# pacellie/raytracer_challenge

Hardware: AMD Instinct MI355X
Metric: Mrays/s (unique rays: primary+shadow+reflection+refraction) at 1920x1080 depth-5 (higher is better)
Workload: dtype f64

## Files before the change

include/rtc.h:

```cpp
#ifndef RTC_H
#define RTC_H
#include <stddef.h>
#include <stdint.h>
#ifdef __cplusplus
extern "C" {
#endif

typedef struct rtc_scene rtc_scene;

enum {
  RTC_OK = 0,
  RTC_ERR_INVALID = 1,
  RTC_ERR_UNSUPPORTED = 2,
  RTC_ERR_DEVICE = 3,
  RTC_ERR_NAN = 4
};

enum { RTC_SPHERE = 0, RTC_PLANE = 1, RTC_CUBE = 2, RTC_CYLINDER = 3, RTC_CONE = 4, RTC_TRIANGLE = 5, RTC_SMOOTH_TRIANGLE = 6 };
enum { RTC_FLAG_CASTS_SHADOW = 1u, RTC_FLAG_CLOSED = 2u };

typedef struct rtc_prim {
  int32_t geometry;
  uint32_t flags;
  int32_t material;
// ... 305 lines not shown
                      uint32_t* order, uint32_t order_cap, uint64_t* keys, uint32_t keys_cap, int32_t* root, double* frame, int32_t* depth, int32_t* stack_need);
int rtc_bvh_collapse_raw(const void* nodes, uint32_t n_nodes, int32_t root, int32_t* depth, int32_t* stack_need);

int rtc_light_grid_build_raw(const int32_t* geometry, const double* limits, const double* transform_inv, const double* tris, uint32_t n_prims, const double* light, int32_t n,
                             int32_t max_list, int32_t tight, uint32_t* cells, uint32_t cells_cap, int32_t* items, uint32_t items_cap, uint32_t* n_items);

int rtc_scan_raw(rtc_scene* scene, uint64_t* values, uint64_t n, uint64_t* total);

enum { RTC_CULL_SLAB = 0, RTC_CULL_POINT = 1, RTC_CULL_GATE = 2, RTC_CULL_PLANE = 3, RTC_CULL_BEHIND = 4 };
int rtc_cull_probe_raw(rtc_scene* scene, int32_t kind, const double* records, uint64_t n, uint8_t* answers);

uint32_t rtc_scene_wavefront_lds_bytes(const rtc_scene*);

int rtc_scene_wavefront_ts_grid(const rtc_scene*, int32_t sync, uint32_t* grid, uint32_t* n_cu, uint32_t* spare_cus, uint32_t* live);

enum { RTC_TRACE_DEFAULT = 0, RTC_TRACE_COUNT = 1, RTC_TRACE_LEAN = 2, RTC_TRACE_3WAVE = 3 };
enum { RTC_WF_TS_MEM = 0, RTC_WF_TS_MEM_COUNT = 1, RTC_WF_TS_LDS = 2, RTC_WF_TS_LDS_COUNT = 3 };
enum { RTC_SHADE_COUNT = 0, RTC_SHADE_COUNT_UV = 1, RTC_SHADE_UV = 2, RTC_SHADE_PIPE_LV0 = 3, RTC_SHADE_PIPE = 4, RTC_SHADE_PAT = 5 };
typedef struct rtc_kernel_info {
  int32_t variant;
  int32_t n_kops;
  int32_t n_kplanes;
  int32_t n_kaux;
  int32_t has_recs;
  int32_t all_plain;
  int32_t no_glass_mirror;
  int32_t big_scene;
  uint32_t lds_bytes;
  int32_t trace_build;
  int32_t wf_ts_build;
// ... 14 lines not shown
```

raytracer_challenge_amd/csrc/device_scene.h:

```cpp
#pragma once
#include <stddef.h>
#include <stdint.h>

enum { OP_PRIM = 0, OP_GROUP = 1, OP_MESH = 2, OP_BVH = 3, OP_QUIRK = 4, OP_QGRID = 5, OP_CSG = 6, OP_CSG_END = 7 };

struct DOp {
  int32_t op, a, b, c;
  int32_t g;
  int32_t pad[3];
};

#define RTC_KOPS 12
#define RTC_KPLANES 6
struct DPlaneK {
  double row[4];
  int32_t prim;
  int32_t gcond;
  int32_t pad[2];
  double n[3];
};

struct DBvhNode {
  float lo0[3], hi0[3];
  float lo1[3], hi1[3];
// ... 216 lines not shown
  unsigned long long bx, by, bz;
  __builtin_memcpy(&bx, &x, 8); __builtin_memcpy(&by, &y, 8); __builtin_memcpy(&bz, &z, 8);
  return rtc_splitmix64(rtc_splitmix64(rtc_splitmix64(rtc_splitmix64((unsigned long long)(uint32_t)light) ^ bx) ^ by) ^ bz);
}
static inline RTC_HD double rtc_area_jitter(unsigned long long h, unsigned j) {
  return (double)(rtc_splitmix64(h ^ (unsigned long long)j) >> 11) * 0x1.0p-53;
}
#define RTC_ALIGHT 16
#define RTC_SLIGHT 22

#define RTC_WF_SHADE_COUNT 32
#define RTC_WF_OVERFLOW 63
#define RTC_WF_CHUNK_NEXT 64
#define RTC_WF_TOP_COUNT (64 + 32 * 8 * (RTC_MAX_FUEL + 2))
#define RTC_WF_SHADE_TOP_COUNT (RTC_WF_TOP_COUNT + 32)
#define RTC_WF_COUNTS (RTC_WF_TOP_COUNT + 64)
#ifndef RTC_WF_CHUNK
#define RTC_WF_CHUNK 64u
#endif
#define RTC_SR_PLAIN 0x40000000
#define RTC_WF_MISS (-2)
struct DWave {
  double* rq[2];
  double* h_t;
  int32_t* h_prim;
  double* h_n12;
  double* sr;
  int32_t* sr_mat;
  int32_t* sr_node;
  double* contrib;
  int32_t* child;
// ... 30 lines not shown
```

raytracer_challenge_amd/csrc/rtc_device.hpp:

```cpp
#pragma once

#include <hip/hip_runtime.h>
#include <stdint.h>

#include <algorithm>
#include <type_traits>

#include "background_point.h"
#include "device_scene.h"
#include "spot_factor.h"

#define EPS 0.00001
#ifndef RTC_BLOCK
#define RTC_BLOCK 64
#endif
#ifndef RTC_WAVES_PER_SIMD
#define RTC_WAVES_PER_SIMD 1
#endif
#ifdef RTC_TRAVERSE_NOINLINE
#define TRAVERSE_INLINE __noinline__
#else
#define TRAVERSE_INLINE __forceinline__
#endif
#ifndef RTC_LANE_ID
// ... 1872 lines not shown
constexpr RtcWfTsBuild rtc_pick_wf_ts_build(bool count, bool lds) { return lds ? (count ? RTC_TS_LDS_COUNT : RTC_TS_LDS) : (count ? RTC_TS_MEM_COUNT : RTC_TS_MEM); }
constexpr unsigned rtc_pick_wf_ts_lds_grid(int n_cu, int spare) {
  return (unsigned)(n_cu < 1 ? 1 : (spare <= 0 ? n_cu : (spare >= n_cu ? 1 : n_cu - spare)));
}
static_assert(rtc_pick_wf_ts_lds_grid(256, 0) == 256u && rtc_pick_wf_ts_lds_grid(256, 24) == 232u && rtc_pick_wf_ts_lds_grid(256, 255) == 1u, "n_cu - spare");
static_assert(rtc_pick_wf_ts_lds_grid(256, 256) == 1u && rtc_pick_wf_ts_lds_grid(256, 261) == 1u && rtc_pick_wf_ts_lds_grid(1, 1) == 1u, "spare >= n_cu: one block");
static_assert(rtc_pick_wf_ts_lds_grid(256, -8) == 256u && rtc_pick_wf_ts_lds_grid(0, 0) == 1u, "a negative spare: n_cu; never an empty grid");
constexpr int rtc_wf_spare_cus_default(int n_cu) { return n_cu < 8 ? 0 : 3 * (n_cu / 8); }
static_assert(rtc_wf_spare_cus_default(256) == 96 && rtc_wf_spare_cus_default(32) == 12 && rtc_wf_spare_cus_default(4) == 0, "3 / 8 of the CUs");
constexpr RtcWfShadeBuild rtc_pick_wf_shade_build(bool count, bool has_uv, bool all_plain, bool level0) {
  if (has_uv) return count ? RTC_SH_COUNT_UV : RTC_SH_UV;
  if (count) return RTC_SH_COUNT;
  if (all_plain) return level0 ? RTC_SH_PIPE_LV0 : RTC_SH_PIPE;
  return RTC_SH_PAT;
}
enum RtcWfShadeNpBuild { RTC_SH_NP = 0, RTC_SH_NP_COUNT = 1, RTC_SH_NP_UV = 2, RTC_SH_NP_COUNT_UV = 3 };
constexpr RtcWfShadeNpBuild rtc_pick_wf_shade_np_build(bool count, bool has_uv) {
  return has_uv ? (count ? RTC_SH_NP_COUNT_UV : RTC_SH_NP_UV) : (count ? RTC_SH_NP_COUNT : RTC_SH_NP);
}

enum RtcExt {
  RTC_EXT_NONE = 0,
  RTC_EXT_BG = 1,
  RTC_EXT_NP = 2,
  RTC_EXT_NP_BG = 3,
};
constexpr int RTC_N_EXT = 4;
constexpr bool rtc_ext_bg(int e) { return (e & RTC_EXT_BG) != 0; }
constexpr bool rtc_ext_np(int e) { return (e & RTC_EXT_NP) != 0; }
static inline RtcExt rtc_ext_of(const RtcSceneExt& X) { return (RtcExt)((X.bg ? RTC_EXT_BG : 0) | (X.bump ? RTC_EXT_NP : 0)); }
// ... 59 lines not shown
```

raytracer_challenge_amd/csrc/rtc_kernels.hip:

```cpp
#include <cstdio>
#include <cstdlib>
#include <utility>

#include "../../include/rtc.h"
#include "rtc_device.hpp"

#ifdef RTC_EMU
#include "rtc_feat.hip"
constexpr int RTC_VARIANTS_BUILT = 6;
#else
constexpr int RTC_VARIANTS_BUILT = RTC_N_VARIANTS;
#endif
template <int... V>
static const RtcVariantOps& rtc_ops(int v, std::integer_sequence<int, V...>) {
  static const RtcVariantOps ops[RTC_N_VARIANTS] = {rtc_variant_ops<V>()...};
  return ops[v];
}
static const RtcVariantOps& rtc_ops(int v) { return rtc_ops(v, std::make_integer_sequence<int, RTC_VARIANTS_BUILT>{}); }
static int rtc_variant(const DScene& S, bool wavefront) {
  return rtc_pick_variant(rtc_scene_feat(S), S.n_kops > 0, S.has_area != 0, S.has_uv != 0, S.has_spot != 0, wavefront);
}

#ifndef RTC_WF_SHADE_WAVES
#define RTC_WF_SHADE_WAVES 4
// ... 13 lines not shown
  const unsigned j = prim >= 0 ? wf_index(parts, W.cap, (unsigned)w) : (first < count ? wf_index(parts, W.cap, (unsigned)first) : 0u);
  WfShadeIn in = {prim, {0.0, 0.0, 0.0, 0.0, 0.0, 0.0}, 1.0, 0.0};
  if (!LV0) in.ray = wf_load_ray(W, level, j, in.weight);
  in.t = W.h_t[j];
  return in;
}
#ifndef RTC_EMU
__device__ __forceinline__ unsigned wf_row_scan16(unsigned v) {
  v += (unsigned)__builtin_amdgcn_update_dpp(0, (int)v, 0x111, 0xf, 0xf, true);
  v += (unsigned)__builtin_amdgcn_update_dpp(0, (int)v, 0x112, 0xf, 0xf, true);
  v += (unsigned)__builtin_amdgcn_update_dpp(0, (int)v, 0x114, 0xf, 0xf, true);
  v += (unsigned)__builtin_amdgcn_update_dpp(0, (int)v, 0x118, 0xf, 0xf, true);
  return v;
}
#endif
}
template <bool COUNT, bool PAT = true, bool UV = false, bool PIPE = false, bool LV0 = false, bool NP = false>
__global__ void __launch_bounds__(RTC_WF_SHADE_BLOCK, RTC_WF_SHADE_WAVES) wf_shade(std::conditional_t<NP, DSceneNp, DScene> S, DCamera cam, DPixelMap pm, DWave W, int level, unsigned n0, int fuel0, DStats* __restrict__ stats) {
  constexpr int end_of[5] = {0, 1, 2, 3, 3};
  constexpr int n_waves = RTC_WF_SHADE_BLOCK >= 64 ? RTC_WF_SHADE_BLOCK / 64 : 1;
  static_assert(n_waves <= 8, "wf_shade: eight counters per class");
  __shared__ unsigned s_cnt2[2][40];
  unsigned parity = 0;
  const WorkMap wm = make_workmap(pm, cam);
  const bool level0 = PIPE ? LV0 : level == 0;
  const WfParts parts = level0 ? WfParts{0u, n0} : wf_count(W, level, n0);
  const unsigned count = parts.top + parts.bottom;
  const size_t cap = W.cap;
  const double L = (double)S.n_lights;
  const int fuel = fuel0 - level;
  unsigned n_reflect = 0, n_refract = 0;
  int32_t* ch = W.child + (size_t)level * 2 * cap;
  double* nq = W.rq[(level + 1) & 1];
  const int lane = RTC_LANE_ID;
  const int wave = (int)(threadIdx.x / (RTC_WF_SHADE_BLOCK >= 64 ? 64 : 1));
  const unsigned long long step = (unsigned long long)gridDim.x * RTC_WF_SHADE_BLOCK;
  WfShadeIn nx = {-1, {0.0, 0.0, 0.0, 0.0, 0.0, 0.0}, 1.0, 0.0};
// ... 39 lines not shown
        if (S.pats[S.mat_pattern[P.mat]].tag != 1) {
          pattern_at<UV>(S, P, st, cr, cg, cbl);
          mat = P.mat;
        }
      }
    }
    const bool blend = hit && reflective > 0.0 && transparency > 0.0;
    double R = 0.0;
    if (blend) {
      R = blend_reflectance(st, n1, n2, fuel, cr, cg, cbl);
      if (R != R && mat < 0) mat = ~mat;
    }
    ChildRays spawn = {false, false, 0.0, 0.0, 0.0, 0.0, 0.0};
    if (hit && fuel > 0) spawn = child_rays(st, n1, n2, weight, L, reflective, transparency, blend, R);
    const unsigned long long lt = (1ull << lane) - 1ull;
    const bool on_plane = hit && geom == 1;
    const unsigned long long m_rec0 = __ballot(hit && on_plane ? 1 : 0), m_rec1 = __ballot(hit && !on_plane ? 1 : 0);
    const unsigned long long m_c0 = __ballot(spawn.refl && on_plane ? 1 : 0), m_c1 = __ballot(spawn.refl && !on_plane ? 1 : 0), m_c2 = __ballot(spawn.refr ? 1 : 0);
    unsigned* s_cnt = s_cnt2[parity];
    parity ^= 1u;
    if (lane == 0) {
      s_cnt[wave] = (unsigned)__popcll(m_rec0); s_cnt[8 + wave] = (unsigned)__popcll(m_rec1);
      s_cnt[16 + wave] = (unsigned)__popcll(m_c0); s_cnt[24 + wave] = (unsigned)__popcll(m_c1); s_cnt[32 + wave] = (unsigned)__popcll(m_c2);
    }
    if (PIPE) nx = wf_shade_prefetch<LV0>(W, parts, level, base + step + threadIdx.x, lane, count, nx_prim);
    __syncthreads();
#ifndef RTC_EMU
    if (PIPE && n_waves == 8 && wave == 0) {
      const unsigned c = lane < 40 ? s_cnt[lane] : 0u;
      const unsigned in_row = wf_row_scan16(c);
      const unsigned r0 = (unsigned)__builtin_amdgcn_readlane((int)in_row, 7), r01 = (unsigned)__builtin_amdgcn_readlane((int)in_row, 15);
      const unsigned k0 = (unsigned)__builtin_amdgcn_readlane((int)in_row, 23), k01 = (unsigned)__builtin_amdgcn_readlane((int)in_row, 31);
      const unsigned k2 = (unsigned)__builtin_amdgcn_readlane((int)in_row, 39);
      const unsigned t_rn = r0, t_rf = r01 - r0, t_cn = k0, t_cf = k01 - k0 + k2;
      const unsigned total = lane == 0 ? t_rn : lane == 1 ? t_rf : lane == 2 ? t_cn : t_cf;
      unsigned first = 0u;
      if (lane < 4 && total) {
        const int row = lane == 0 ? RTC_WF_SHADE_COUNT + level : lane == 1 ? RTC_WF_SHADE_TOP_COUNT + level : lane == 2 ? level + 1 : RTC_WF_TOP_COUNT + level + 1;
        const unsigned old = atomicAdd(&W.counts[row], total);
        const bool fits = (unsigned long long)old + total <= W.cap;
        if (!fits) { W.counts[RTC_WF_OVERFLOW] = 1u; stats->wf_overflow = 1ull; }
        first = (lane & 1) ? (fits ? W.cap - old - total : W.cap) : old;
      }
      const unsigned b_rn = (unsigned)__builtin_amdgcn_readlane((int)first, 0), b_rf = (unsigned)__builtin_amdgcn_readlane((int)first, 1);
      const unsigned b_cn = (unsigned)__builtin_amdgcn_readlane((int)first, 2), b_cf = (unsigned)__builtin_amdgcn_readlane((int)first, 3);
      if (lane < 40) {
        const unsigned ex = in_row - c;
        s_cnt[lane] = lane < 8 ? b_rn + ex : lane < 16 ? b_rf + ex - r0 : lane < 24 ? b_cn + ex : lane < 32 ? b_cf + ex - k0 : b_cf + k01 - k0 + ex;
      }
    }
    if (!PIPE || n_waves != 8)
#endif
    if (threadIdx.x == 0) {
      unsigned t[4] = {0u, 0u, 0u, 0u}, b[4];
      for (int k = 0; k < 5; k++)
        for (int w = 0; w < n_waves; w++) t[end_of[k]] += s_cnt[8 * k + w];
      const int row[4] = {RTC_WF_SHADE_COUNT + level, RTC_WF_SHADE_TOP_COUNT + level, level + 1, RTC_WF_TOP_COUNT + level + 1};
      for (int e = 0; e < 4; e++) {
        const unsigned old = t[e] ? atomicAdd(&W.counts[row[e]], t[e]) : 0u;
        const bool fits = (unsigned long long)old + t[e] <= W.cap;
        if (!fits) { W.counts[RTC_WF_OVERFLOW] = 1u; stats->wf_overflow = 1ull; }
        b[e] = (e & 1) ? (fits ? W.cap - old - t[e] : W.cap) : old;
      }
      for (int k = 0; k < 5; k++)
        for (int w = 0; w < n_waves; w++) { const unsigned r = s_cnt[8 * k + w]; s_cnt[8 * k + w] = b[end_of[k]]; b[end_of[k]] += r; }
    }
    __syncthreads();
    const unsigned s = on_plane ? s_cnt[wave] + (unsigned)__popcll(m_rec0 & lt) : s_cnt[8 + wave] + (unsigned)__popcll(m_rec1 & lt);
    const unsigned jr = on_plane ? s_cnt[16 + wave] + (unsigned)__popcll(m_c0 & lt) : s_cnt[24 + wave] + (unsigned)__popcll(m_c1 & lt);
    const unsigned jt = s_cnt[32 + wave] + (unsigned)__popcll(m_c2 & lt);
    if (hit && s < W.cap) {
      double* r = W.sr;
      r[s] = st.px; r[cap + s] = st.py; r[2 * cap + s] = st.pz;
      r[3 * cap + s] = st.nx; r[4 * cap + s] = st.ny; r[5 * cap + s] = st.nz;
      if (mat >= 0) {
        r[6 * cap + s] = cr; r[7 * cap + s] = cg; r[8 * cap + s] = cbl;
        W.sr_mat[s] = mat;
      } else {
        if (!PIPE) shading_row = (int)S.mat[8 * ~mat + 7];
        W.sr_mat[s] = RTC_SR_PLAIN | shading_row;
      }
      W.sr_node[s] = (int32_t)i;
    }
// ... 86 lines not shown
}
int rtc_ext_trace_build(const DScene& S, const RtcSceneExt& X) {
  return X.bump ? rtc_pick_np_build(S.has_area != 0, S.has_uv != 0, S.has_spot != 0, X.bg != nullptr) : rtc_pick_bg_build(S.has_area != 0, S.has_uv != 0, S.has_spot != 0);
}
bool rtc_scene_is_big(unsigned long long scene_bytes) { return rtc_big_scene(scene_bytes); }

#ifndef RTC_EMU

unsigned rtc_wavefront_grid(const DScene& S, int n_cu) {
  return (unsigned)std::max(1, n_cu * rtc_ops(rtc_variant(S, true)).wf_ts_blocks_per_cu(rtc_stack_bytes(S)));
}
unsigned rtc_wavefront_lds_grid(int n_cu, int spare) { return rtc_pick_wf_ts_lds_grid(n_cu, spare); }
int rtc_wavefront_spare_cus_default(int n_cu) { return rtc_wf_spare_cus_default(n_cu); }
#endif

uint64_t rtc_wavefront_work(const DCamera& cam, const DPixelMap& pm) {
  if (pm.mode == 2 && cam.hsize >= 8 && pm.n % cam.hsize == 0) return (uint64_t)((cam.hsize + 7) / 8) * ((pm.n / cam.hsize + 7) / 8) * 64;
  return pm.n;
}

#ifndef RTC_EMU
void rtc_launch_wf_background(const DScene& S, const DCamera& cam, const DPixelMap& pm, const DWave& W, int level, unsigned n0, const DBackground& bg, unsigned blocks,
                              hipStream_t stream);
#endif
void rtc_launch_wavefront(const DScene& S, const DCamera& cam, const DPixelMap& pm, int fuel, const DWave& W, double* rgb, double* hit_t, int* hit_prim, int* hit_k,
                          DStats* stats, bool count, hipStream_t stream, unsigned blocks, unsigned shade_blocks, unsigned lds, unsigned lds_blocks, const RtcSceneExt& X) {
  if (pm.n == 0) return;
  const RtcVariantOps& ops = rtc_ops(rtc_variant(S, true));
  const RtcFrame F = {S, cam, pm, hit_t, hit_prim, hit_k, stats, stream, count};
  const unsigned n0 = (unsigned)rtc_wavefront_work(cam, pm);
  const dim3 sgrid(std::max(1u, shade_blocks)), sblock(RTC_WF_SHADE_BLOCK);
  auto shade = [&](auto kernel, const auto& scene, int level) { hipLaunchKernelGGL(kernel, sgrid, sblock, 0, stream, scene, cam, pm, W, level, n0, fuel, stats); };
#ifndef RTC_EMU
  DSceneNp N;
  if (X.bump) N = rtc_widen_scene(S, X);
#endif
  for (int level = 0; level <= fuel + 1; level++) {
    const int tl = level <= fuel ? level : -1, sl = level - 1;
#ifndef RTC_EMU
    if (!lds || !ops.launch_wf_ts_lds(F, RtcLevel{W, tl, sl, n0, level, fuel - level, std::max(1u, lds_blocks), lds}))
#endif
    ops.launch_wf_ts(F, RtcLevel{W, tl, sl, n0, level, fuel - level, blocks, 0u});
    if (level > fuel) break;
#ifndef RTC_EMU
    if (X.bg) rtc_launch_wf_background(S, cam, pm, W, level, n0, *X.bg, 4u * std::max(1u, shade_blocks), stream);
    if (X.bump) {
      switch (rtc_pick_wf_shade_np_build(count, S.has_uv != 0)) {
        case RTC_SH_NP_COUNT_UV: shade(wf_shade<true, true, true, false, false, true>, N, level); break;
        case RTC_SH_NP_UV: shade(wf_shade<false, true, true, false, false, true>, N, level); break;
        case RTC_SH_NP_COUNT: shade(wf_shade<true, true, false, false, false, true>, N, level); break;
        case RTC_SH_NP: shade(wf_shade<false, true, false, false, false, true>, N, level); break;
      }
      continue;
    }
#endif
    switch (rtc_scene_shade_build(S, count, level == 0)) {
#ifndef RTC_EMU
      case RTC_SH_COUNT_UV: shade(wf_shade<true, true, true>, S, level); break;
      case RTC_SH_UV: shade(wf_shade<false, true, true>, S, level); break;
#else
      case RTC_SH_COUNT_UV: case RTC_SH_UV: break;
#endif
      case RTC_SH_COUNT: shade(wf_shade<true>, S, level); break;
      case RTC_SH_PIPE_LV0: shade(wf_shade<false, false, false, true, true>, S, level); break;
      case RTC_SH_PIPE: shade(wf_shade<false, false, false, true, false>, S, level); break;
      case RTC_SH_PAT: shade(wf_shade<false>, S, level); break;
    }
  }
  hipLaunchKernelGGL(wf_gather, dim3(std::max(1u, std::min(blocks, (n0 + 255u) / 256u))), dim3(256), 0, stream, cam, pm, W, n0, rgb);
}
void rtc_launch_wavefront(const DScene& S, const DCamera& cam, const DPixelMap& pm, int fuel, const DWave& W, double* rgb, double* hit_t, int* hit_prim, int* hit_k,
                          DStats* stats, bool count, hipStream_t stream, unsigned blocks, unsigned shade_blocks) {
  rtc_launch_wavefront(S, cam, pm, fuel, W, rgb, hit_t, hit_prim, hit_k, stats, count, stream, blocks, shade_blocks, 0u, 0u, RtcSceneExt{nullptr, nullptr});
}

static dim3 rtc_elementwise_grid(unsigned long long n) { return dim3((unsigned)std::min<unsigned long long>((n + 255) / 256, 8192)); }
__global__ void __launch_bounds__(256) rtc_quantize_kernel(const double* __restrict__ rgb, unsigned char* __restrict__ out, unsigned long long n) {
  unsigned long long i = (unsigned long long)blockIdx.x * blockDim.x + threadIdx.x;
  const unsigned long long stride = (unsigned long long)gridDim.x * blockDim.x;
  for (; i < n; i += stride) {
    double x = rgb[i];
    double c = (x != x) ? 1.0 : (x < 1.0 ? x : 1.0);
    c = c > 0.0 ? c : 0.0;
    double r = round(c * 255.0);
    out[i] = (unsigned char)(r <= 0.0 ? 0.0 : (r >= 255.0 ? 255.0 : r));
  }
}
__global__ void __launch_bounds__(256) rtc_pack_hits_kernel(const double* __restrict__ t, const int* __restrict__ prim, const int* __restrict__ k, DHit* __restrict__ out, unsigned long long n) {
// ... 49 lines not shown
```

raytracer_challenge_amd/csrc/rtc_scene.cpp:

```cpp
#include <hip/hip_runtime_api.h>

#include <algorithm>
#include <atomic>
#include <chrono>
#include <cmath>
#include <condition_variable>
#include <cstdlib>
#include <cstdio>
#include <cstring>
#include <deque>
#include <functional>
#include <initializer_list>
#include <memory>
#include <mutex>
#include <string>
#include <thread>
#include <vector>

#include "../../include/rtc.h"
#include "adaptive_contrast.h"
#include "background_point.h"
#include "bump_normal.h"
#include "camera_sampling.h"
#include "device_scene.h"
#include "filter_weights.h"
#include "scene_build.hpp"
#include "shutter_pose.h"
#include "spot_factor.h"
#include "uv_image.h"

void rtc_launch_trace(const DScene& S, const DCamera& cam, const DPixelMap& pm, int fuel, double* rgb, double* hit_t, int* hit_prim, int* hit_k,
                      DStats* stats, bool count, hipStream_t stream, bool big_scene, const RtcSceneExt& X);
void rtc_launch_quantize(const double* rgb, unsigned char* out, unsigned long long n, hipStream_t stream);
void rtc_launch_pack_hits(const double* t, const int* prim, const int* k, DHit* out, unsigned long long n, hipStream_t stream);
void rtc_launch_deinterleave(const double* slab, double* image, unsigned rowlen, unsigned vsize, unsigned n, unsigned max_rows, unsigned band, hipStream_t stream);
void rtc_launch_deinterleave8(const unsigned char* slab, unsigned char* image, unsigned rowlen, unsigned vsize, unsigned n, unsigned max_rows, unsigned band, hipStream_t stream);
void rtc_launch_wavefront(const DScene& S, const DCamera& cam, const DPixelMap& pm, int fuel, const DWave& W, double* rgb, double* hit_t, int* hit_prim, int* hit_k,
                          DStats* stats, bool count, hipStream_t stream, unsigned blocks, unsigned shade_blocks, unsigned lds, unsigned lds_blocks, const RtcSceneExt& X);
void rtc_launch_bump_normals(const DScene& S, const DBumpTable& bt, const int32_t* prims, const double* points, const double* normals, unsigned long long n, double* out,
                             hipStream_t stream);
void rtc_launch_background_colors(const DScene& S, const DBackground& bg, const double* dirs, unsigned long long n, double* rgb, hipStream_t stream);
int rtc_ext_trace_build(const DScene& S, const RtcSceneExt& X);
void rtc_kernel_info_fill(const DScene& S, bool wavefront, bool count, bool big_scene, unsigned lds_bytes, int device, rtc_kernel_info* out);
bool rtc_scene_is_big(unsigned long long scene_bytes);
uint64_t rtc_wavefront_work(const DCamera& cam, const DPixelMap& pm);
unsigned rtc_wavefront_grid(const DScene& S, int n_cu);
unsigned rtc_wavefront_lds_grid(int n_cu, int spare);
int rtc_wavefront_spare_cus_default(int n_cu);
unsigned rtc_wavefront_lds_bytes(const DScene& S, bool enabled);
void rtc_launch_gen_rays(const DCamera& cam, const DPixelMap& pm, const rtc_sampling& sp, unsigned long long slot_first, unsigned long long n_slots, double* rays,
                         hipStream_t stream);
void rtc_launch_resolve_samples(const double* ray_rgb, unsigned n_samples, unsigned long long n_slots, double* dst, hipStream_t stream);
unsigned long long rtc_contrast_blocks(unsigned long long n);
// ... 78 lines not shown
  int tune_n[2] = {0, 0};
  int tune_choice = 0;
  uint32_t n_analytic = 0;
  uint32_t n_bouncing = 0;
  uint32_t n_prims_total = 0;
  bool last_wavefront = false;
  int last_fuel = 0;
  DCsgHit* csg_slab = nullptr;
  uint64_t csg_slab_threads = 0;
  bool wave_alloc_failed = false;
  DWave wave{};
  void* wave_mem = nullptr;
  uint64_t wave_cap = 0;
  int wave_levels = 0;
  unsigned wave_blocks = 0, shade_blocks = 0;
  unsigned lds_bytes = 0;
  int n_cu = 1;
  int spare_cus = 0;
  bool counted = false;
  unsigned wave_eighths = 9;
  int bvh_depth = 0;
  int built_on_device = 0;
  uint32_t n_bvh_nodes = 0, n_mesh_tris = 0;

  template <class T>
  int upload(const std::vector<T>& v, const T** out) {
    *out = nullptr;
    if (v.empty()) return RTC_OK;
    void* p = nullptr;
    HIP_OK(hipMalloc(&p, v.size() * sizeof(T)));
// ... 179 lines not shown
      if (tuned) drop_wavefront(s);
      else s->wave_alloc_failed = true;
      return run(s, cam, pm, fuel, d_rgb, want_hits, stats, count, sync, 1, after);
    }
    if (rc != RTC_OK) return rc;
    s->wave.dig = nullptr;
    if (pm.digest && count) {
      const uint64_t need = (uint64_t)s->wave_cap * (uint64_t)(fuel + 1);
      rc = grow(&s->cap_wave_dig, need, {{(void**)&s->d_wave_dig, need * sizeof(unsigned long long)}}, s->stream);
      if (rc != RTC_OK) return rc;
      s->wave.dig = s->d_wave_dig;
    }
    HIP_OK(hipMemsetAsync(s->wave.counts, 0, RTC_WF_COUNTS * sizeof(uint32_t), s->stream));
    HIP_OK(hipEventRecord(s->ev0, s->stream));
    rtc_launch_wavefront(s->d, cam, pm, fuel, s->wave, d_rgb, want_hits ? s->d_hit_t : nullptr, s->d_hit_prim, s->d_hit_k, s->d_stats, count, s->stream, s->wave_blocks, s->shade_blocks, s->lds_bytes,
                         lds_grid(s, will_sync), s->ext());
  } else {
    rtc_launch_trace(s->d, cam, pm, fuel, d_rgb, want_hits ? s->d_hit_t : nullptr, s->d_hit_prim, s->d_hit_k, s->d_stats, count, s->stream, rtc_scene_is_big(s->bytes), s->ext());
  }
  HIP_OK(hipGetLastError());
  HIP_OK(hipEventRecord(s->ev1, s->stream));
  s->last_wavefront = wavefront;
  s->last_fuel = fuel;
  if (after) { int rca = (*after)(); if (rca != RTC_OK) return rca; }
  if (!sync && !stats) return RTC_OK;
  HIP_OK(hipStreamSynchronize(s->stream));
  DStats h;
  int rcs = read_clear_sticky(s, &h);
  if (rcs != RTC_OK) return rcs;
  if (wavefront) {
    if (std::getenv("RTC_WF_DUMP_COUNTS")) {
// ... 698 lines not shown
    };
    bool ok = verify("items", d.item_prim, H.items.data(), H.items.size() * 4);
    ok = verify("qcell", d.qcell, H.qcell.data(), H.qcell.size() * 4) && ok;
    ok = verify("ops", d.ops, H.ops.data(), H.ops.size() * sizeof(DOp)) && ok;
    std::fprintf(stderr, "[rtc] upload verify: %s; n_items=%zu n_qcell=%zu n_prims=%zu\n", ok ? "ok" : "MISMATCH", H.items.size(), H.qcell.size(), H.prims.size());
  }
  if (timing) std::fprintf(stderr, "[rtc-timing] %-28s %.3f s (%.1f MB)\n", "upload", std::chrono::duration<double>(std::chrono::steady_clock::now() - t_up0).count(), (double)s->bytes / 1e6);
  HIP_OK(hipMalloc((void**)&s->d_stats, sizeof(DStats)));
  HIP_OK(hipMemset(s->d_stats, 0, sizeof(DStats)));
  {
    const char* kv = std::getenv("RTC_KERNEL");
    const int kvi = kv ? std::atoi(kv) : 0;
    s->kernel_version = (kvi == 1 || kvi == 4) ? kvi : 0;
    const char* le = std::getenv("RTC_WF_LDS");
    s->lds_bytes = rtc_wavefront_lds_bytes(s->d, !(le && le[0] == '0'));
    int n_cu = 0;
    HIP_OK(hipDeviceGetAttribute(&n_cu, hipDeviceAttributeMultiprocessorCount, device));
    s->wave_blocks = rtc_wavefront_grid(s->d, n_cu);
    if (const char* w = std::getenv("RTC_WF_BLOCKS_PER_CU")) s->wave_blocks = (unsigned)std::max(1, n_cu * std::atoi(w));
    s->shade_blocks = (unsigned)std::max(1, n_cu * 2);
    if (const char* w = std::getenv("RTC_WF_SHADE_BLOCKS_PER_CU")) s->shade_blocks = (unsigned)std::max(1, n_cu * std::atoi(w));
    s->n_cu = std::max(1, n_cu);
    const char* sp = std::getenv("RTC_WF_SPARE_CUS");
    s->spare_cus = std::min(std::max(sp ? std::atoi(sp) : rtc_wavefront_spare_cus_default(s->n_cu), 0), s->n_cu - 1);
  }
  if (device >= 0 && device < RTC_LIVE_DEVICES) {
    g_live_scenes[device].fetch_add(1, std::memory_order_relaxed);
    s->counted = true;
  }
  *out = s.release();
// ... 1033 lines not shown
  hipError_t e = hipMemcpyAsync(d, records, rec_bytes, hipMemcpyHostToDevice, s->stream);
  if (e == hipSuccess) {
    rtc_launch_cull_probe(kind, (const double*)d, n, d + rec_bytes, s->stream);
    e = hipGetLastError();
  }
  if (e == hipSuccess) e = hipMemcpyAsync(answers, d + rec_bytes, n, hipMemcpyDeviceToHost, s->stream);
  const hipError_t e_sync = hipStreamSynchronize(s->stream);
  (void)hipFree(d);
  HIP_OK(e);
  HIP_OK(e_sync);
  return RTC_OK;
}

uint32_t rtc_scene_wavefront_lds_bytes(const rtc_scene* s) { return s ? s->lds_bytes : 0u; }

int rtc_scene_wavefront_ts_grid(const rtc_scene* s, int32_t sync, uint32_t* grid, uint32_t* n_cu, uint32_t* spare_cus, uint32_t* live) {
  if (!s) return rtc_fail(RTC_ERR_INVALID, "NULL argument");
  if (grid) *grid = s->lds_bytes ? lds_grid(s, sync != 0) : s->wave_blocks;
  if (n_cu) *n_cu = (uint32_t)s->n_cu;
  if (spare_cus) *spare_cus = (uint32_t)s->spare_cus;
  if (live) *live = (uint32_t)live_scenes(s->device);
  return RTC_OK;
}

int rtc_scene_kernel_info(const rtc_scene* s, int32_t path, int32_t count, rtc_kernel_info* out) {
  if (!s || !out) return rtc_fail(RTC_ERR_INVALID, "NULL argument");
  if (path != 1 && path != 4) return rtc_fail(RTC_ERR_INVALID, "path must be 1 (one kernel) or 4 (wavefront)");
  rtc_kernel_info_fill(s->d, path == 4, count != 0, rtc_scene_is_big(s->bytes), s->lds_bytes, s->device, out);
  return RTC_OK;
}
// ... 10 lines not shown
```

raytracer_challenge_amd/device.py:

```python
from __future__ import annotations

import ctypes as C

from .backend import Backend, CameraC, NativeWorld, RtwError, SamplingC
from .scene import Camera, Sampling


class RtcCameraC(C.Structure):
    _fields_ = [("hsize", C.c_uint64), ("vsize", C.c_uint64), ("half_width", C.c_double), ("half_height", C.c_double),
                ("pixel_size", C.c_double), ("transform_inv", C.c_double * 16)]


class RtcStatsC(C.Structure):
    _COUNTERS = ("pixels", "rays_primary", "rays_shadow", "rays_reflect", "rays_refract", "rays_container",
                 "accel_nodes", "group_tests", "tri_tests", "analytic_tests", "nan_ts")
    _fields_ = [(n, C.c_uint64) for n in _COUNTERS] + \
               [("kernel_ms", C.c_double), ("n_launches", C.c_uint32), ("_pad", C.c_uint32),
                ("accel_nodes_kernarg", C.c_uint64), ("analytic_tests_kernarg", C.c_uint64), ("light_grid_cells", C.c_uint64),
                ("group_tests_uniform", C.c_uint64)]

    def as_dict(self):
        d = {n: int(getattr(self, n)) for n in self._COUNTERS + ("accel_nodes_kernarg", "analytic_tests_kernarg", "light_grid_cells", "group_tests_uniform")}
        d["kernel_ms"] = float(self.kernel_ms)
        d["n_launches"] = int(self.n_launches)
# ... 139 lines not shown
        lib.rtc_scene_path_info.restype = None
        lib.rtc_scene_path_info.argtypes = [C.c_void_p, C.POINTER(C.c_int32), C.POINTER(C.c_double), C.POINTER(C.c_double)]
        ch, a, b = C.c_int32(0), C.c_double(-1), C.c_double(-1)
        lib.rtc_scene_path_info(self.scene, C.byref(ch), C.byref(a), C.byref(b))
        return {"path": {0: "undecided", 1: "one kernel", 4: "wavefront"}.get(ch.value, str(ch.value)),
                "one_kernel_ms": a.value, "wavefront_ms": b.value}

    def wavefront_grid(self, sync: bool) -> dict:
        lib = self.backend.lib
        lib.rtc_scene_wavefront_ts_grid.restype = C.c_int
        lib.rtc_scene_wavefront_ts_grid.argtypes = [C.c_void_p, C.c_int32] + [C.POINTER(C.c_uint32)] * 4
        a = [C.c_uint32(0) for _ in range(4)]
        self._rc(lib.rtc_scene_wavefront_ts_grid(self.scene, 1 if sync else 0, *[C.byref(x) for x in a]), "rtc_scene_wavefront_ts_grid")
        return {"grid": a[0].value, "n_cu": a[1].value, "spare_cus": a[2].value, "live_scenes": a[3].value}

    def info(self) -> dict:
        a = [C.c_uint32(0) for _ in range(4)]
        self.backend.lib.rtc_scene_accel_info(self.scene, *[C.byref(x) for x in a])
        return {"scene_device_bytes": int(self.backend.lib.rtc_scene_device_bytes(self.scene)), "program_ops": a[0].value,
                "bvh_nodes": a[1].value, "mesh_triangles": a[2].value, "bvh_depth": a[3].value,
                "wavefront_lds_bytes_per_block": int(self.backend.lib.rtc_scene_wavefront_lds_bytes(self.scene))}
```

Measured before the change: 13410.

## Sort non-plane shade records by primitive into bins for wavefront levels

New measurement: 13170. -1.8%, worse.

```diff
diff --git a/include/rtc.h b/include/rtc.h
--- a/include/rtc.h
+++ b/include/rtc.h
@@ -343,6 +343,10 @@
 
 int rtc_scene_wavefront_ts_grid(const rtc_scene*, int32_t sync, uint32_t* grid, uint32_t* n_cu, uint32_t* spare_cus, uint32_t* live);
 
+uint32_t rtc_scene_wavefront_bins(const rtc_scene*);
+
+int rtc_scene_wavefront_last_records(rtc_scene*, int32_t* prims, uint64_t cap, uint32_t* n_far, uint32_t* n_near);
+
 enum { RTC_TRACE_DEFAULT = 0, RTC_TRACE_COUNT = 1, RTC_TRACE_LEAN = 2, RTC_TRACE_3WAVE = 3 };
 enum { RTC_WF_TS_MEM = 0, RTC_WF_TS_MEM_COUNT = 1, RTC_WF_TS_LDS = 2, RTC_WF_TS_LDS_COUNT = 3 };
 enum { RTC_SHADE_COUNT = 0, RTC_SHADE_COUNT_UV = 1, RTC_SHADE_UV = 2, RTC_SHADE_PIPE_LV0 = 3, RTC_SHADE_PIPE = 4, RTC_SHADE_PAT = 5 };
diff --git a/raytracer_challenge_amd/csrc/device_scene.h b/raytracer_challenge_amd/csrc/device_scene.h
--- a/raytracer_challenge_amd/csrc/device_scene.h
+++ b/raytracer_challenge_amd/csrc/device_scene.h
@@ -254,7 +254,10 @@
 #define RTC_WF_CHUNK_NEXT 64
 #define RTC_WF_TOP_COUNT (64 + 32 * 8 * (RTC_MAX_FUEL + 2))
 #define RTC_WF_SHADE_TOP_COUNT (RTC_WF_TOP_COUNT + 32)
-#define RTC_WF_COUNTS (RTC_WF_TOP_COUNT + 64)
+#define RTC_WF_BINS 1024
+#define RTC_WF_BIN_HIST (RTC_WF_TOP_COUNT + 64)
+#define RTC_WF_BIN_CURSOR (RTC_WF_BIN_HIST + 2 * RTC_WF_BINS)
+#define RTC_WF_COUNTS (RTC_WF_BIN_CURSOR + 2 * RTC_WF_BINS)
 #ifndef RTC_WF_CHUNK
 #define RTC_WF_CHUNK 64u
 #endif
diff --git a/raytracer_challenge_amd/csrc/rtc_device.hpp b/raytracer_challenge_amd/csrc/rtc_device.hpp
--- a/raytracer_challenge_amd/csrc/rtc_device.hpp
+++ b/raytracer_challenge_amd/csrc/rtc_device.hpp
@@ -1910,6 +1910,10 @@
   if (all_plain) return level0 ? RTC_SH_PIPE_LV0 : RTC_SH_PIPE;
   return RTC_SH_PAT;
 }
+constexpr unsigned rtc_pick_wf_bins(int n_prims, bool enabled) { return enabled && n_prims >= 1 && n_prims <= RTC_WF_BINS ? (unsigned)n_prims : 0u; }
+static_assert(rtc_pick_wf_bins(0, true) == 0u && rtc_pick_wf_bins(1, true) == 1u && rtc_pick_wf_bins(1024, true) == 1024u && rtc_pick_wf_bins(1025, true) == 0u,
+              "bins: 1 .. RTC_WF_BINS primitives");
+static_assert(rtc_pick_wf_bins(64, false) == 0u && rtc_pick_wf_bins(-1, true) == 0u, "bins: off by the switch; never a negative count");
 enum RtcWfShadeNpBuild { RTC_SH_NP = 0, RTC_SH_NP_COUNT = 1, RTC_SH_NP_UV = 2, RTC_SH_NP_COUNT_UV = 3 };
 constexpr RtcWfShadeNpBuild rtc_pick_wf_shade_np_build(bool count, bool has_uv) {
   return has_uv ? (count ? RTC_SH_NP_COUNT_UV : RTC_SH_NP_UV) : (count ? RTC_SH_NP_COUNT : RTC_SH_NP);
diff --git a/raytracer_challenge_amd/csrc/rtc_kernels.hip b/raytracer_challenge_amd/csrc/rtc_kernels.hip
--- a/raytracer_challenge_amd/csrc/rtc_kernels.hip
+++ b/raytracer_challenge_amd/csrc/rtc_kernels.hip
@@ -51,13 +51,76 @@
   return v;
 }
 #endif
-}
-template <bool COUNT, bool PAT = true, bool UV = false, bool PIPE = false, bool LV0 = false, bool NP = false>
+#define WF_ON_PLANE(geom) ((geom) == 1)
+__device__ __forceinline__ uint32_t* wf_bin_hist(const DWave& W, int level) { return W.counts + RTC_WF_BIN_HIST + RTC_WF_BINS * (level & 1); }
+__device__ __forceinline__ uint32_t* wf_bin_cursor(const DWave& W, int level) { return W.counts + RTC_WF_BIN_CURSOR + RTC_WF_BINS * (level & 1); }
+constexpr int WF_SHADE_WAVE = RTC_WF_SHADE_BLOCK >= 64 ? 64 : 1;
+constexpr int WF_SHADE_N_WAVES = RTC_WF_SHADE_BLOCK / WF_SHADE_WAVE;
+__device__ __forceinline__ void wf_bin_prefix(const uint32_t* __restrict__ hist, unsigned n_bins, unsigned* prefix, unsigned* wsum) {
+  constexpr unsigned K = RTC_WF_BINS / RTC_WF_SHADE_BLOCK;
+  static_assert(K * RTC_WF_SHADE_BLOCK == RTC_WF_BINS, "wf_bin_prefix: every thread the same number of bins");
+  const int lane = RTC_LANE_ID, wave = (int)(threadIdx.x / WF_SHADE_WAVE);
+  const unsigned b0 = threadIdx.x * K;
+  unsigned v = 0u;
+  for (unsigned k = 0; k < K; k++) v += b0 + k < n_bins ? hist[b0 + k] : 0u;
+  unsigned inc = v;
+  for (int d = 1; d < WF_SHADE_WAVE; d <<= 1) {
+    const unsigned o = __shfl(inc, lane >= d ? lane - d : lane);
+    if (lane >= d) inc += o;
+  }
+  if (lane == WF_SHADE_WAVE - 1) wsum[wave] = inc;
+  __syncthreads();
+  unsigned run = inc - v;
+  for (int w = 0; w < wave; w++) run += wsum[w];
+  for (unsigned k = 0; k < K; k++) {
+    prefix[b0 + k] = run;
+    run += b0 + k < n_bins ? hist[b0 + k] : 0u;
+  }
+  __syncthreads();
+}
+}
+__global__ void __launch_bounds__(RTC_WF_SHADE_BLOCK) wf_bin_count(const DPrim* __restrict__ prims, DWave W, int level, unsigned n0, unsigned n_bins) {
+  __shared__ unsigned s_hist[RTC_WF_BINS];
+  __shared__ unsigned char s_plane[RTC_WF_BINS];
+  __shared__ unsigned s_total;
+  if (n_bins > RTC_WF_BINS) n_bins = RTC_WF_BINS;
+  for (unsigned b = threadIdx.x; b < n_bins; b += RTC_WF_SHADE_BLOCK) { s_hist[b] = 0u; s_plane[b] = WF_ON_PLANE(prims[b].geom) ? 1 : 0; }
+  if (threadIdx.x == 0) s_total = 0u;
+  const unsigned long long step = (unsigned long long)gridDim.x * RTC_WF_SHADE_BLOCK, first = (unsigned long long)blockIdx.x * RTC_WF_SHADE_BLOCK + threadIdx.x;
+  uint32_t* other_hist = wf_bin_hist(W, level + 1);
+  uint32_t* other_cursor = wf_bin_cursor(W, level + 1);
+  for (unsigned long long b = first; b < RTC_WF_BINS; b += step) { other_hist[b] = 0u; other_cursor[b] = 0u; }
+  __syncthreads();
+  const WfParts parts = wf_count(W, level, n0);
+  const unsigned count = parts.top + parts.bottom;
+  for (unsigned long long w = first; w < count; w += step) {
+    const int prim = W.h_prim[wf_index(parts, W.cap, (unsigned)w)];
+    if (prim >= 0 && (unsigned)prim < n_bins && !s_plane[prim]) atomicAdd(&s_hist[prim], 1u);
+  }
+  __syncthreads();
+  uint32_t* hist = wf_bin_hist(W, level);
+  unsigned mine = 0u;
+  for (unsigned b = threadIdx.x; b < n_bins; b += RTC_WF_SHADE_BLOCK) {
+    const unsigned c = s_hist[b];
+    if (c) { atomicAdd(&hist[b], c); mine += c; }
+  }
+  if (mine) atomicAdd(&s_total, mine);
+  __syncthreads();
+  if (threadIdx.x == 0 && s_total) atomicAdd(&W.counts[RTC_WF_SHADE_TOP_COUNT + level], s_total);
+}
+template <bool COUNT, bool PAT = true, bool UV = false, bool PIPE = false, bool LV0 = false, bool NP = false, bool BIN = false>
 __global__ void __launch_bounds__(RTC_WF_SHADE_BLOCK, RTC_WF_SHADE_WAVES) wf_shade(std::conditional_t<NP, DSceneNp, DScene> S, DCamera cam, DPixelMap pm, DWave W, int level, unsigned n0, int fuel0, DStats* __restrict__ stats) {
   constexpr int end_of[5] = {0, 1, 2, 3, 3};
   constexpr int n_waves = RTC_WF_SHADE_BLOCK >= 64 ? RTC_WF_SHADE_BLOCK / 64 : 1;
   static_assert(n_waves <= 8, "wf_shade: eight counters per class");
   __shared__ unsigned s_cnt2[2][40];
+  __shared__ unsigned s_bin_prefix[BIN ? RTC_WF_BINS : 1], s_bin_n[BIN ? RTC_WF_BINS : 1], s_bin_base[BIN ? RTC_WF_BINS : 1], s_bin_wsum[8];
+  unsigned bin_total = 0u;
+  if constexpr (BIN) {
+    bin_total = W.counts[RTC_WF_SHADE_TOP_COUNT + level];
+    for (unsigned b = threadIdx.x; b < RTC_WF_BINS; b += RTC_WF_SHADE_BLOCK) s_bin_n[b] = 0u;
+    wf_bin_prefix(wf_bin_hist(W, level), (unsigned)S.n_prims, s_bin_prefix, s_bin_wsum);
+  }
   unsigned parity = 0;
   const WorkMap wm = make_workmap(pm, cam);
   const bool level0 = PIPE ? LV0 : level == 0;
@@ -127,7 +190,7 @@
     ChildRays spawn = {false, false, 0.0, 0.0, 0.0, 0.0, 0.0};
     if (hit && fuel > 0) spawn = child_rays(st, n1, n2, weight, L, reflective, transparency, blend, R);
     const unsigned long long lt = (1ull << lane) - 1ull;
-    const bool on_plane = hit && geom == 1;
+    const bool on_plane = hit && WF_ON_PLANE(geom);
     const unsigned long long m_rec0 = __ballot(hit && on_plane ? 1 : 0), m_rec1 = __ballot(hit && !on_plane ? 1 : 0);
     const unsigned long long m_c0 = __ballot(spawn.refl && on_plane ? 1 : 0), m_c1 = __ballot(spawn.refl && !on_plane ? 1 : 0), m_c2 = __ballot(spawn.refr ? 1 : 0);
     unsigned* s_cnt = s_cnt2[parity];
@@ -136,8 +199,19 @@
       s_cnt[wave] = (unsigned)__popcll(m_rec0); s_cnt[8 + wave] = (unsigned)__popcll(m_rec1);
       s_cnt[16 + wave] = (unsigned)__popcll(m_c0); s_cnt[24 + wave] = (unsigned)__popcll(m_c1); s_cnt[32 + wave] = (unsigned)__popcll(m_c2);
     }
+    const bool binned = BIN && hit && !on_plane && (unsigned)prim < RTC_WF_BINS;
+    unsigned rank = 0u;
+    if constexpr (BIN) if (binned) rank = atomicAdd(&s_bin_n[prim], 1u);
     if (PIPE) nx = wf_shade_prefetch<LV0>(W, parts, level, base + step + threadIdx.x, lane, count, nx_prim);
     __syncthreads();
+    unsigned bin_base = 0u;
+    if constexpr (BIN) {
+      if (binned && rank == 0u) {
+        const unsigned n = s_bin_n[prim];
+        s_bin_n[prim] = 0u;
+        bin_base = atomicAdd(&wf_bin_cursor(W, level)[prim], n);
+      }
+    }
 #ifndef RTC_EMU
     if (PIPE && n_waves == 8 && wave == 0) {
       const unsigned c = lane < 40 ? s_cnt[lane] : 0u;
@@ -145,7 +219,7 @@
       const unsigned r0 = (unsigned)__builtin_amdgcn_readlane((int)in_row, 7), r01 = (unsigned)__builtin_amdgcn_readlane((int)in_row, 15);
       const unsigned k0 = (unsigned)__builtin_amdgcn_readlane((int)in_row, 23), k01 = (unsigned)__builtin_amdgcn_readlane((int)in_row, 31);
       const unsigned k2 = (unsigned)__builtin_amdgcn_readlane((int)in_row, 39);
-      const unsigned t_rn = r0, t_rf = r01 - r0, t_cn = k0, t_cf = k01 - k0 + k2;
+      const unsigned t_rn = r0, t_rf = BIN ? 0u : r01 - r0, t_cn = k0, t_cf = k01 - k0 + k2;
       const unsigned total = lane == 0 ? t_rn : lane == 1 ? t_rf : lane == 2 ? t_cn : t_cf;
       unsigned first = 0u;
       if (lane < 4 && total) {
@@ -167,7 +241,7 @@
     if (threadIdx.x == 0) {
       unsigned t[4] = {0u, 0u, 0u, 0u}, b[4];
       for (int k = 0; k < 5; k++)
-        for (int w = 0; w < n_waves; w++) t[end_of[k]] += s_cnt[8 * k + w];
+        for (int w = 0; w < n_waves; w++) if (!(BIN && k == 1)) t[end_of[k]] += s_cnt[8 * k + w];
       const int row[4] = {RTC_WF_SHADE_COUNT + level, RTC_WF_SHADE_TOP_COUNT + level, level + 1, RTC_WF_TOP_COUNT + level + 1};
       for (int e = 0; e < 4; e++) {
         const unsigned old = t[e] ? atomicAdd(&W.counts[row[e]], t[e]) : 0u;
@@ -178,8 +252,14 @@
       for (int k = 0; k < 5; k++)
         for (int w = 0; w < n_waves; w++) { const unsigned r = s_cnt[8 * k + w]; s_cnt[8 * k + w] = b[end_of[k]]; b[end_of[k]] += r; }
     }
+    if constexpr (BIN) if (binned && rank == 0u) s_bin_base[prim] = bin_base;
     __syncthreads();
-    const unsigned s = on_plane ? s_cnt[wave] + (unsigned)__popcll(m_rec0 & lt) : s_cnt[8 + wave] + (unsigned)__popcll(m_rec1 & lt);
+    unsigned s_bin = W.cap;
+    if constexpr (BIN) {
+      const unsigned off = binned ? s_bin_prefix[prim] + s_bin_base[prim] + rank : bin_total;
+      if (bin_total <= W.cap && off < bin_total) s_bin = W.cap - bin_total + off;
+    }
+    const unsigned s = BIN && !on_plane ? s_bin : on_plane ? s_cnt[wave] + (unsigned)__popcll(m_rec0 & lt) : s_cnt[8 + wave] + (unsigned)__popcll(m_rec1 & lt);
     const unsigned jr = on_plane ? s_cnt[16 + wave] + (unsigned)__popcll(m_c0 & lt) : s_cnt[24 + wave] + (unsigned)__popcll(m_c1 & lt);
     const unsigned jt = s_cnt[32 + wave] + (unsigned)__popcll(m_c2 & lt);
     if (hit && s < W.cap) {
@@ -296,6 +376,15 @@
 int rtc_wavefront_spare_cus_default(int n_cu) { return rtc_wf_spare_cus_default(n_cu); }
 #endif
 
+unsigned rtc_wavefront_bins(const DScene& S, const RtcSceneExt& X, bool enabled) {
+#ifdef RTC_EMU
+  const bool uv = false;
+#else
+  const bool uv = S.has_uv != 0;
+#endif
+  return rtc_pick_wf_bins(S.n_prims, enabled && !uv && !X.bump);
+}
+
 uint64_t rtc_wavefront_work(const DCamera& cam, const DPixelMap& pm) {
   if (pm.mode == 2 && cam.hsize >= 8 && pm.n % cam.hsize == 0) return (uint64_t)((cam.hsize + 7) / 8) * ((pm.n / cam.hsize + 7) / 8) * 64;
   return pm.n;
@@ -306,8 +395,9 @@
                               hipStream_t stream);
 #endif
 void rtc_launch_wavefront(const DScene& S, const DCamera& cam, const DPixelMap& pm, int fuel, const DWave& W, double* rgb, double* hit_t, int* hit_prim, int* hit_k,
-                          DStats* stats, bool count, hipStream_t stream, unsigned blocks, unsigned shade_blocks, unsigned lds, unsigned lds_blocks, const RtcSceneExt& X) {
+                          DStats* stats, bool count, hipStream_t stream, unsigned blocks, unsigned shade_blocks, unsigned lds, unsigned lds_blocks, const RtcSceneExt& X, bool bins) {
   if (pm.n == 0) return;
+  const unsigned n_bins = rtc_wavefront_bins(S, X, bins);
   const RtcVariantOps& ops = rtc_ops(rtc_variant(S, true));
   const RtcFrame F = {S, cam, pm, hit_t, hit_prim, hit_k, stats, stream, count};
   const unsigned n0 = (unsigned)rtc_wavefront_work(cam, pm);
@@ -324,6 +414,8 @@
 #endif
     ops.launch_wf_ts(F, RtcLevel{W, tl, sl, n0, level, fuel - level, blocks, 0u});
     if (level > fuel) break;
+    const bool binned = n_bins != 0u && level >= 1;
+    if (binned) hipLaunchKernelGGL(wf_bin_count, dim3(std::max(1u, shade_blocks / 2u)), sblock, 0, stream, S.prims, W, level, n0, n_bins);
 #ifndef RTC_EMU
     if (X.bg) rtc_launch_wf_background(S, cam, pm, W, level, n0, *X.bg, 4u * std::max(1u, shade_blocks), stream);
     if (X.bump) {
@@ -343,17 +435,27 @@
 #else
       case RTC_SH_COUNT_UV: case RTC_SH_UV: break;
 #endif
-      case RTC_SH_COUNT: shade(wf_shade<true>, S, level); break;
+      case RTC_SH_COUNT:
+        if (binned) shade(wf_shade<true, true, false, false, false, false, true>, S, level);
+        else shade(wf_shade<true>, S, level);
+        break;
       case RTC_SH_PIPE_LV0: shade(wf_shade<false, false, false, true, true>, S, level); break;
-      case RTC_SH_PIPE: shade(wf_shade<false, false, false, true, false>, S, level); break;
-      case RTC_SH_PAT: shade(wf_shade<false>, S, level); break;
+      case RTC_SH_PIPE:
+        if (binned) shade(wf_shade<false, false, false, true, false, false, true>, S, level);
+        else shade(wf_shade<false, false, false, true, false>, S, level);
+        break;
+      case RTC_SH_PAT:
+        if (binned) shade(wf_shade<false, true, false, false, false, false, true>, S, level);
+        else shade(wf_shade<false>, S, level);
+        break;
     }
   }
   hipLaunchKernelGGL(wf_gather, dim3(std::max(1u, std::min(blocks, (n0 + 255u) / 256u))), dim3(256), 0, stream, cam, pm, W, n0, rgb);
 }
 void rtc_launch_wavefront(const DScene& S, const DCamera& cam, const DPixelMap& pm, int fuel, const DWave& W, double* rgb, double* hit_t, int* hit_prim, int* hit_k,
                           DStats* stats, bool count, hipStream_t stream, unsigned blocks, unsigned shade_blocks) {
-  rtc_launch_wavefront(S, cam, pm, fuel, W, rgb, hit_t, hit_prim, hit_k, stats, count, stream, blocks, shade_blocks, 0u, 0u, RtcSceneExt{nullptr, nullptr});
+  const char* be = std::getenv("RTC_WF_BINS");
+  rtc_launch_wavefront(S, cam, pm, fuel, W, rgb, hit_t, hit_prim, hit_k, stats, count, stream, blocks, shade_blocks, 0u, 0u, RtcSceneExt{nullptr, nullptr}, !(be && be[0] == '0'));
 }
 
 static dim3 rtc_elementwise_grid(unsigned long long n) { return dim3((unsigned)std::min<unsigned long long>((n + 255) / 256, 8192)); }
diff --git a/raytracer_challenge_amd/csrc/rtc_scene.cpp b/raytracer_challenge_amd/csrc/rtc_scene.cpp
--- a/raytracer_challenge_amd/csrc/rtc_scene.cpp
+++ b/raytracer_challenge_amd/csrc/rtc_scene.cpp
@@ -36,7 +36,8 @@
 void rtc_launch_deinterleave(const double* slab, double* image, unsigned rowlen, unsigned vsize, unsigned n, unsigned max_rows, unsigned band, hipStream_t stream);
 void rtc_launch_deinterleave8(const unsigned char* slab, unsigned char* image, unsigned rowlen, unsigned vsize, unsigned n, unsigned max_rows, unsigned band, hipStream_t stream);
 void rtc_launch_wavefront(const DScene& S, const DCamera& cam, const DPixelMap& pm, int fuel, const DWave& W, double* rgb, double* hit_t, int* hit_prim, int* hit_k,
-                          DStats* stats, bool count, hipStream_t stream, unsigned blocks, unsigned shade_blocks, unsigned lds, unsigned lds_blocks, const RtcSceneExt& X);
+                          DStats* stats, bool count, hipStream_t stream, unsigned blocks, unsigned shade_blocks, unsigned lds, unsigned lds_blocks, const RtcSceneExt& X, bool bins);
+unsigned rtc_wavefront_bins(const DScene& S, const RtcSceneExt& X, bool enabled);
 void rtc_launch_bump_normals(const DScene& S, const DBumpTable& bt, const int32_t* prims, const double* points, const double* normals, unsigned long long n, double* out,
                              hipStream_t stream);
 void rtc_launch_background_colors(const DScene& S, const DBackground& bg, const double* dirs, unsigned long long n, double* rgb, hipStream_t stream);
@@ -145,6 +146,7 @@
   uint64_t wave_cap = 0;
   int wave_levels = 0;
   unsigned wave_blocks = 0, shade_blocks = 0;
+  bool wf_bins = true;
   unsigned lds_bytes = 0;
   int n_cu = 1;
   int spare_cus = 0;
@@ -354,7 +356,7 @@
     HIP_OK(hipMemsetAsync(s->wave.counts, 0, RTC_WF_COUNTS * sizeof(uint32_t), s->stream));
     HIP_OK(hipEventRecord(s->ev0, s->stream));
     rtc_launch_wavefront(s->d, cam, pm, fuel, s->wave, d_rgb, want_hits ? s->d_hit_t : nullptr, s->d_hit_prim, s->d_hit_k, s->d_stats, count, s->stream, s->wave_blocks, s->shade_blocks, s->lds_bytes,
-                         lds_grid(s, will_sync), s->ext());
+                         lds_grid(s, will_sync), s->ext(), s->wf_bins);
   } else {
     rtc_launch_trace(s->d, cam, pm, fuel, d_rgb, want_hits ? s->d_hit_t : nullptr, s->d_hit_prim, s->d_hit_k, s->d_stats, count, s->stream, rtc_scene_is_big(s->bytes), s->ext());
   }
@@ -1083,6 +1085,8 @@
     s->kernel_version = (kvi == 1 || kvi == 4) ? kvi : 0;
     const char* le = std::getenv("RTC_WF_LDS");
     s->lds_bytes = rtc_wavefront_lds_bytes(s->d, !(le && le[0] == '0'));
+    const char* be = std::getenv("RTC_WF_BINS");
+    s->wf_bins = !(be && be[0] == '0');
     int n_cu = 0;
     HIP_OK(hipDeviceGetAttribute(&n_cu, hipDeviceAttributeMultiprocessorCount, device));
     s->wave_blocks = rtc_wavefront_grid(s->d, n_cu);
@@ -2146,6 +2150,32 @@
 
 uint32_t rtc_scene_wavefront_lds_bytes(const rtc_scene* s) { return s ? s->lds_bytes : 0u; }
 
+uint32_t rtc_scene_wavefront_bins(const rtc_scene* s) { return s ? rtc_wavefront_bins(s->d, s->ext(), s->wf_bins) : 0u; }
+
+int rtc_scene_wavefront_last_records(rtc_scene* s, int32_t* prims, uint64_t cap, uint32_t* n_far, uint32_t* n_near) {
+  if (!s || !n_far || !n_near || (!prims && cap)) return rtc_fail(RTC_ERR_INVALID, "NULL argument");
+  if (!s->last_wavefront || !s->wave_mem) return rtc_fail(RTC_ERR_INVALID, "the scene's most recent launch was not a wavefront launch");
+  HIP_OK(hipSetDevice(s->device));
+  HIP_OK(hipStreamSynchronize(s->stream));
+  const uint64_t qcap = s->wave_cap;
+  uint32_t far = 0, near = 0;
+  HIP_OK(hipMemcpy(&far, s->wave.counts + RTC_WF_SHADE_TOP_COUNT + s->last_fuel, sizeof(far), hipMemcpyDeviceToHost));
+  HIP_OK(hipMemcpy(&near, s->wave.counts + RTC_WF_SHADE_COUNT + s->last_fuel, sizeof(near), hipMemcpyDeviceToHost));
+  far = (uint32_t)std::min<uint64_t>(far, qcap);
+  near = (uint32_t)std::min<uint64_t>(near, qcap - far);
+  *n_far = far; *n_near = near;
+  if ((uint64_t)far + near > cap) return rtc_fail(RTC_ERR_INVALID, "more shade records than the caller's buffer holds");
+  std::vector<int32_t> node(qcap), prim(qcap);
+  HIP_OK(hipMemcpy(node.data(), s->wave.sr_node, qcap * sizeof(int32_t), hipMemcpyDeviceToHost));
+  HIP_OK(hipMemcpy(prim.data(), s->wave.h_prim, qcap * sizeof(int32_t), hipMemcpyDeviceToHost));
+  for (uint64_t k = 0; k < (uint64_t)far + near; k++) {
+    const uint64_t slot = k < far ? qcap - far + k : k - far;
+    const int32_t ray = node[slot];
+    prims[k] = ray >= 0 && (uint64_t)ray < qcap ? prim[ray] : -1;
+  }
+  return RTC_OK;
+}
+
 int rtc_scene_wavefront_ts_grid(const rtc_scene* s, int32_t sync, uint32_t* grid, uint32_t* n_cu, uint32_t* spare_cus, uint32_t* live) {
   if (!s) return rtc_fail(RTC_ERR_INVALID, "NULL argument");
   if (grid) *grid = s->lds_bytes ? lds_grid(s, sync != 0) : s->wave_blocks;
diff --git a/raytracer_challenge_amd/device.py b/raytracer_challenge_amd/device.py
--- a/raytracer_challenge_amd/device.py
+++ b/raytracer_challenge_amd/device.py
@@ -177,6 +177,26 @@
         self._rc(lib.rtc_scene_wavefront_ts_grid(self.scene, 1 if sync else 0, *[C.byref(x) for x in a]), "rtc_scene_wavefront_ts_grid")
         return {"grid": a[0].value, "n_cu": a[1].value, "spare_cus": a[2].value, "live_scenes": a[3].value}
 
+    def wavefront_bins(self) -> int:
+        lib = self.backend.lib
+        lib.rtc_scene_wavefront_bins.restype = C.c_uint32
+        lib.rtc_scene_wavefront_bins.argtypes = [C.c_void_p]
+        return int(lib.rtc_scene_wavefront_bins(self.scene))
+
+    def wavefront_last_records(self) -> tuple:
+        import numpy as np
+        lib = self.backend.lib
+        lib.rtc_scene_wavefront_last_records.restype = C.c_int
+        lib.rtc_scene_wavefront_last_records.argtypes = [C.c_void_p, C.c_void_p, C.c_uint64, C.POINTER(C.c_uint32), C.POINTER(C.c_uint32)]
+        n_far, n_near = C.c_uint32(0), C.c_uint32(0)
+        prims = np.empty(0, dtype=np.int32)
+        rc = lib.rtc_scene_wavefront_last_records(self.scene, None, 0, C.byref(n_far), C.byref(n_near))
+        if n_far.value + n_near.value > 0:
+            prims = np.empty(n_far.value + n_near.value, dtype=np.int32)
+            rc = lib.rtc_scene_wavefront_last_records(self.scene, prims.ctypes.data, len(prims), C.byref(n_far), C.byref(n_near))
+        self._rc(rc, "rtc_scene_wavefront_last_records")
+        return prims[:n_far.value].copy(), prims[n_far.value:n_far.value + n_near.value].copy()
+
     def info(self) -> dict:
         a = [C.c_uint32(0) for _ in range(4)]
         self.backend.lib.rtc_scene_accel_info(self.scene, *[C.byref(x) for x in a])
```
